# borodark/exmc

Hardware: AMD Instinct MI355X
Metric: leapfrog_steps_per_s (higher is better)
Workload: dtype f64; 1 GPU; eight_schools d=10, 4096 chains/GPU (4096 total), 138450 draws/chain (2769 steps of 50 draws) after one shared 1000-iteration warmup, max_tree_depth 10, target_accept 0.8; draws_per_chain=138450, lanes_per_chain=16, warmup_lanes_per_chain=16, seed=42

## Files before the change

exmc_amd/csrc/exmc_device.hpp:

```cpp
#pragma once

#include <hip/hip_runtime.h>
#include <stdint.h>
#include <type_traits>

#include <utility>

#include "../../include/exmc_detmath.h"

namespace exmc {

constexpr uint64_t kMask58 = (1ULL << 58) - 1;

__device__ __forceinline__ bool div_in_range(double x) {
  const uint32_t h = (uint32_t)__double2hiint(x) & 0x7fffffffu;
  return (h - 0x28300000u) < (0x57C00000u - 0x28300000u);
}

struct Recip {
  double b, r;
};

__device__ __forceinline__ Recip make_recip(double b) { return Recip{b, exmc_rcp_refined(b)}; }

__device__ __forceinline__ Recip make_recip_literal(double b) {
  __asm__ volatile("" : "+v"(b));
  return make_recip(b);
// ... 250 lines not shown
#define EXMC_SEQ2(I) EXMC_SEQ1(I) EXMC_FMAC_B(a1, v1, I)
#define EXMC_SEQ3(I) EXMC_SEQ2(I) EXMC_FMAC_B(a2, v2, I)
#define EXMC_SEQ6(I) EXMC_SEQ3(I) EXMC_FMAC_B(a3, v3, I) EXMC_FMAC_B(a4, v4, I) EXMC_FMAC_B(a5, v5, I)
#define EXMC_LANES_1(S) S(0)
#define EXMC_LANES_2(S) EXMC_LANES_1(S) S(1)
#define EXMC_LANES_3(S) EXMC_LANES_2(S) S(2)
#define EXMC_LANES_4(S) EXMC_LANES_3(S) S(3)
#define EXMC_LANES_5(S) EXMC_LANES_4(S) S(4)
#define EXMC_LANES_6(S) EXMC_LANES_5(S) S(5)
#define EXMC_LANES_7(S) EXMC_LANES_6(S) S(6)
#define EXMC_LANES_8(S) EXMC_LANES_7(S) S(7)
#define EXMC_LANES_9(S) EXMC_LANES_8(S) S(8)
#define EXMC_LANES_10(S) EXMC_LANES_9(S) S(9)
#define EXMC_LANES_11(S) EXMC_LANES_10(S) S(10)
#define EXMC_LANES_12(S) EXMC_LANES_11(S) S(11)
#define EXMC_SEQSUM_ASM(SEQ, OUTS, INS)                                                        \
  if constexpr (NL == 1) __asm__("s_nop 1\n\t" EXMC_LANES_1(SEQ) : OUTS : INS);                \
  else if constexpr (NL == 2) __asm__("s_nop 1\n\t" EXMC_LANES_2(SEQ) : OUTS : INS);           \
  else if constexpr (NL == 3) __asm__("s_nop 1\n\t" EXMC_LANES_3(SEQ) : OUTS : INS);           \
  else if constexpr (NL == 4) __asm__("s_nop 1\n\t" EXMC_LANES_4(SEQ) : OUTS : INS);           \
  else if constexpr (NL == 5) __asm__("s_nop 1\n\t" EXMC_LANES_5(SEQ) : OUTS : INS);           \
  else if constexpr (NL == 6) __asm__("s_nop 1\n\t" EXMC_LANES_6(SEQ) : OUTS : INS);           \
  else if constexpr (NL == 7) __asm__("s_nop 1\n\t" EXMC_LANES_7(SEQ) : OUTS : INS);           \
  else if constexpr (NL == 8) __asm__("s_nop 1\n\t" EXMC_LANES_8(SEQ) : OUTS : INS);           \
  else if constexpr (NL == 9) __asm__("s_nop 1\n\t" EXMC_LANES_9(SEQ) : OUTS : INS);           \
  else if constexpr (NL == 10) __asm__("s_nop 1\n\t" EXMC_LANES_10(SEQ) : OUTS : INS);         \
  else if constexpr (NL == 11) __asm__("s_nop 1\n\t" EXMC_LANES_11(SEQ) : OUTS : INS);         \
  else __asm__("s_nop 1\n\t" EXMC_LANES_12(SEQ) : OUTS : INS);
#define EXMC_COMMA ,

__device__ __forceinline__ double seq_one() { return 1.0; }

template <int NL>
__device__ __forceinline__ void row_seqsum(double& a0, double v0) {
  static_assert(NL >= 1 && NL <= 12, "lanes of one DPP row, where the chain beats the butterfly");
  const double one = seq_one();
  EXMC_SEQSUM_ASM(EXMC_SEQ1, [a0] "+v"(a0), [v0] "v"(v0) EXMC_COMMA [one] "v"(one))
}
template <int NL>
__device__ __forceinline__ void row_seqsum(double& a0, double& a1, double v0, double v1) {
  const double one = seq_one();
  EXMC_SEQSUM_ASM(EXMC_SEQ2, [a0] "+v"(a0) EXMC_COMMA [a1] "+v"(a1),
                  [v0] "v"(v0) EXMC_COMMA [v1] "v"(v1) EXMC_COMMA [one] "v"(one))
}
template <int NL>
__device__ __forceinline__ void row_seqsum(double& a0, double& a1, double& a2, double v0, double v1,
                                           double v2) {
  const double one = seq_one();
  EXMC_SEQSUM_ASM(EXMC_SEQ3, [a0] "+v"(a0) EXMC_COMMA [a1] "+v"(a1) EXMC_COMMA [a2] "+v"(a2),
                  [v0] "v"(v0) EXMC_COMMA [v1] "v"(v1) EXMC_COMMA [v2] "v"(v2) EXMC_COMMA [one] "v"(one))
}
#define EXMC_FMAC_R(A, V, I) \
  "v_fmac_f64_dpp %[" #A "], %[" #V "], %[one] row_newbcast:%[l" #I "] row_mask:0xf bank_mask:0xf\n\t"
#define EXMC_SEQ3R(I) EXMC_FMAC_R(a0, v0, I) EXMC_FMAC_R(a1, v1, I) EXMC_FMAC_R(a2, v2, I)
#define EXMC_LANE_R(I) [l##I] "n"((I0 + I) & 15)
template <int I0, int NL>
__device__ __forceinline__ void row_seqsum_lanes(double& a0, double& a1, double& a2, double v0, double v1,
                                                 double v2) {
  static_assert(I0 >= 0 && NL >= 1 && NL <= 12 && I0 + NL <= 16, "a lane range of one DPP row");
  const double one = seq_one();
  EXMC_SEQSUM_ASM(EXMC_SEQ3R, [a0] "+v"(a0) EXMC_COMMA [a1] "+v"(a1) EXMC_COMMA [a2] "+v"(a2),
                  [v0] "v"(v0) EXMC_COMMA [v1] "v"(v1) EXMC_COMMA [v2] "v"(v2) EXMC_COMMA [one] "v"(one) EXMC_COMMA
                  EXMC_LANE_R(0) EXMC_COMMA EXMC_LANE_R(1) EXMC_COMMA EXMC_LANE_R(2) EXMC_COMMA EXMC_LANE_R(3) EXMC_COMMA
                  EXMC_LANE_R(4) EXMC_COMMA EXMC_LANE_R(5) EXMC_COMMA EXMC_LANE_R(6) EXMC_COMMA EXMC_LANE_R(7) EXMC_COMMA
                  EXMC_LANE_R(8) EXMC_COMMA EXMC_LANE_R(9) EXMC_COMMA EXMC_LANE_R(10) EXMC_COMMA EXMC_LANE_R(11))
}
#ifndef EXMC_ROW_SUM_PIECES
#define EXMC_ROW_SUM_PIECES 7
#endif
#define EXMC_MV1(I) \
  "v_fmac_f64_dpp %[acc], %[x], %[c" #I "] row_newbcast:" #I " row_mask:0xf bank_mask:0xf\n\t"
template <int NL>
__device__ __forceinline__ double row_matvec(double x, const double (&c)[NL]) {
  static_assert(NL >= 1 && NL <= 12, "lanes of one DPP row");
  double acc = 0.0;
#define EXMC_MV_C(I) [c##I] "v"(c[(I) < NL ? (I) : 0])
  EXMC_SEQSUM_ASM(EXMC_MV1, [acc] "+v"(acc),
                  [x] "v"(x) EXMC_COMMA EXMC_MV_C(0) EXMC_COMMA EXMC_MV_C(1) EXMC_COMMA EXMC_MV_C(2) EXMC_COMMA
                  EXMC_MV_C(3) EXMC_COMMA EXMC_MV_C(4) EXMC_COMMA EXMC_MV_C(5) EXMC_COMMA EXMC_MV_C(6) EXMC_COMMA
                  EXMC_MV_C(7) EXMC_COMMA EXMC_MV_C(8) EXMC_COMMA EXMC_MV_C(9) EXMC_COMMA EXMC_MV_C(10) EXMC_COMMA
                  EXMC_MV_C(11))
#undef EXMC_MV_C
  return acc;
}
#define EXMC_OUTER1(I) \
  "v_fmac_f64_dpp %[m" #I "], %[x], %[c] row_newbcast:" #I " row_mask:0xf bank_mask:0xf\n\t"
template <int NL>
__device__ __forceinline__ void row_outer_acc(double (&m)[NL], double x, double c) {
  static_assert(NL >= 1 && NL <= 12, "lanes of one DPP row");
  double pad[12];
#pragma unroll
  for (int j = 0; j < 12; j++) pad[j] = (j < NL) ? m[j < NL ? j : 0] : 0.0;
#define EXMC_OUTER_M(I) [m##I] "+v"(pad[I])
  EXMC_SEQSUM_ASM(EXMC_OUTER1,
                  EXMC_OUTER_M(0) EXMC_COMMA EXMC_OUTER_M(1) EXMC_COMMA EXMC_OUTER_M(2) EXMC_COMMA EXMC_OUTER_M(3) EXMC_COMMA
                  EXMC_OUTER_M(4) EXMC_COMMA EXMC_OUTER_M(5) EXMC_COMMA EXMC_OUTER_M(6) EXMC_COMMA EXMC_OUTER_M(7) EXMC_COMMA
                  EXMC_OUTER_M(8) EXMC_COMMA EXMC_OUTER_M(9) EXMC_COMMA EXMC_OUTER_M(10) EXMC_COMMA EXMC_OUTER_M(11),
                  [x] "v"(x) EXMC_COMMA [c] "v"(c))
#undef EXMC_OUTER_M
#pragma unroll
  for (int j = 0; j < NL; j++) m[j] = pad[j];
}
template <int J>
__device__ __forceinline__ double row_bcast_f64(double x) {
  double acc = 0.0;
  const double one = seq_one();
  __asm__("s_nop 1\n\tv_fmac_f64_dpp %0, %1, %2 row_newbcast:%3 row_mask:0xf bank_mask:0xf"
          : "+v"(acc) : "v"(x), "v"(one), "n"(J));
  return acc;
}

template <int NL>
__device__ __forceinline__ void row_seqsum6(double (&a)[6], const double (&v)[6]) {
  const double one = seq_one();
  EXMC_SEQSUM_ASM(EXMC_SEQ6,
                  [a0] "+v"(a[0]) EXMC_COMMA [a1] "+v"(a[1]) EXMC_COMMA [a2] "+v"(a[2]) EXMC_COMMA
                  [a3] "+v"(a[3]) EXMC_COMMA [a4] "+v"(a[4]) EXMC_COMMA [a5] "+v"(a[5]),
                  [v0] "v"(v[0]) EXMC_COMMA [v1] "v"(v[1]) EXMC_COMMA [v2] "v"(v[2]) EXMC_COMMA
                  [v3] "v"(v[3]) EXMC_COMMA [v4] "v"(v[4]) EXMC_COMMA [v5] "v"(v[5]) EXMC_COMMA
                  [one] "v"(one))
}

template <int G>
__device__ __forceinline__ double group_bcast(double v, int src) {
  if (G == 1) return v;
  const int lane = threadIdx.x & 63;
  return __shfl(v, (lane & ~(G - 1)) | src, 64);
}

template <int G, int SRC>
__device__ __forceinline__ double group_bcast_c(double v) {
  static_assert(SRC >= 0 && SRC < G, "source lane outside the group");
  if constexpr (G == 1) {
    return v;
  } else if constexpr (G == 2) {
// ... 213 lines not shown
    const double mx = (a > b) ? a : b;
    if (mx == -exmc_from_bits(EXMC_INF_BITS) || mx == -1.0e300) return -1.0e300;
    const double mn = (a > b) ? b : a;
    return mx + log_ge1(1.0 + exp_le0(mn - mx));
  }
  __device__ static __forceinline__ double lse_arg(double a, double b) {
    return ((a > b) ? b : a) - ((a > b) ? a : b);
  }
  __device__ static __forceinline__ double lse_finish(double a, double b, double log1pe) {
    const double mx = (a > b) ? a : b;
    const bool none = (mx == -exmc_from_bits(EXMC_INF_BITS) || mx == -1.0e300);
    return none ? -1.0e300 : mx + log1pe;
  }
};

template <int CTRL>
__device__ __forceinline__ double xchg_dpp(double v) { return dpp_move<CTRL>(v); }
template <int PATTERN>
__device__ __forceinline__ double xchg_swizzle(double v) {
  return __hiloint2double(__builtin_amdgcn_ds_swizzle(__double2hiint(v), PATTERN),
                          __builtin_amdgcn_ds_swizzle(__double2loint(v), PATTERN));
}
__device__ __forceinline__ double xchg_xor4(double v) {
#if EXMC_XROW_PERMLANE
  return __hiloint2double(xor4_b32(__double2hiint(v)), xor4_b32(__double2loint(v)));
#else
  return xchg_swizzle<(4 << 10) | 0x1F>(v);
#endif
}
__device__ __forceinline__ double xchg_xor32(double v) {
// ... 133 lines not shown
#pragma unroll
  for (int k = 0; k < DPL; k++) {
    const double v = rho[k] * im[k];
    sa = valid[k] ? (sa + v * pa[k]) : sa;
    sb = valid[k] ? (sb + v * pb[k]) : sb;
  }
}

template <int G, int DPL, int D = G * DPL, bool kLds = false>
__device__ __forceinline__ bool uturn(const double (&rho)[DPL], const double (&pa)[DPL],
                                      const double (&pb)[DPL], const double (&im)[DPL],
                                      const bool (&valid)[DPL]) {
  double s[2];
  if constexpr (kSeqSum<G, D>) {
    const double v = rho[0] * im[0];
    s[0] = s[1] = 0.0;
    row_seqsum<D>(s[0], s[1], v * pa[0], v * pb[0]);
  } else {
    uturn_partials<DPL>(rho, pa, pb, im, valid, s[0], s[1]);
    if constexpr (G == 64 && (kLds || EXMC_XROW_PERMLANE)) {
      const unsigned long long neg = __ballot((rs64_reduce2(s) < 0.0) ? 1 : 0);
      return (neg & 0x3ULL) != 0;
    } else {
      group_allsum_n<G, 2, kLds>(s);
    }
  }
  return (s[0] < 0.0) || (s[1] < 0.0);
}

template <int G, int DPL, int D = G * DPL, bool kLds = false>
__device__ __forceinline__ void uturn3(const double (&r1)[DPL], const double (&a1)[DPL],
                                       const double (&b1)[DPL], const double (&r2)[DPL],
                                       const double (&a2)[DPL], const double (&b2)[DPL],
                                       const double (&r3)[DPL], const double (&a3)[DPL],
                                       const double (&b3)[DPL], const double (&im)[DPL],
                                       const bool (&valid)[DPL], bool& c1, bool& c23) {
  double s[6];
  if constexpr (kSeqSum<G, D>) {
    const double v1 = r1[0] * im[0], v2 = r2[0] * im[0], v3 = r3[0] * im[0];
    const double t[6] = {v1 * a1[0], v1 * b1[0], v2 * a2[0], v2 * b2[0], v3 * a3[0], v3 * b3[0]};
#pragma unroll
    for (int j = 0; j < 6; j++) s[j] = 0.0;
    row_seqsum6<D>(s, t);
  } else {
    uturn_partials<DPL>(r1, a1, b1, im, valid, s[0], s[1]);
    uturn_partials<DPL>(r2, a2, b2, im, valid, s[2], s[3]);
    uturn_partials<DPL>(r3, a3, b3, im, valid, s[4], s[5]);
    if constexpr (G == 64 && (kLds || EXMC_XROW_PERMLANE)) {
      const unsigned long long neg = __ballot((rs64_reduce6(s) < 0.0) ? 1 : 0);
      c1 = (neg & ((1ULL << 0) | (1ULL << 4))) != 0;
      c23 = (neg & ((1ULL << 1) | (1ULL << 2) | (1ULL << 3) | (1ULL << 5))) != 0;
      return;
    } else {
      group_allsum_n<G, 6, kLds>(s);
    }
  }
  c1 = (s[0] < 0.0) || (s[1] < 0.0);
  c23 = (s[2] < 0.0) || (s[3] < 0.0) || (s[4] < 0.0) || (s[5] < 0.0);
// ... 232 lines not shown
```

exmc_amd/csrc/exmc_hip.hip:

```cpp
#include "../../include/exmc_hip.h"
#include "../../include/exmc_hip_compare.h"
#include "../../include/exmc_hip_pathfinder.h"
#include "../../include/exmc_hip_advi.h"
#include "../../include/exmc_hip_predictive.h"
#include "../../include/exmc_hip_ppc.h"
#include "../../include/exmc_hip_loo_pit.h"
#include "../../include/exmc_hip_convergence.h"

#include <hip/hip_runtime.h>

#include <cmath>
#include <cstdio>
#include <cstdlib>
#include <cstring>
#include <algorithm>
#include <atomic>
#include <mutex>
#include <string>
#include <type_traits>
#include <unordered_map>
#include <vector>

#include "../../include/exmc_zig_tables.h"
#include "exmc_kernels.hpp"
// ... 20 lines not shown
  if (e != hipSuccess) return e;
  e = hipMemcpyToSymbol(HIP_SYMBOL(g_prof), z, sizeof(z));
  if (e != hipSuccess) return e;
  static const char* nm[9] = {"transition_start", "doubling_start", "leapfrog+model", "leaf",
                              "ascend", "outer_merge", "transition_done", "tree_prefix", "loop"};
  unsigned long long tot = 0;
  for (int i = 0; i < 9; i++) tot += h[i];
  fprintf(stderr, "[exmc prof] %s %.3f ms, passes (sum over waves) %llu, cycles %llu\n", what, ms, h[9], tot);
  for (int i = 0; i < 9; i++)
    if ((i != 7 || h[7]) && h[9])
      fprintf(stderr, "[exmc prof]   %-18s %6.1f%%  %8.1f cycles/pass\n", nm[i],
              100.0 * (double)h[i] / (double)tot, (double)h[i] / (double)h[9]);
  if (h[10])
    fprintf(stderr, "[exmc prof]   integrator wave: %llu units, %.1f cycles/unit compute, %.1f barrier wait, %.1f other\n",
            h[10], (double)h[11] / (double)h[10], (double)h[12] / (double)h[10], (double)h[13] / (double)h[10]);
  return hipSuccess;
}
#endif


const uint64_t kZigKi[256] = EXMC_ZIG_KI_INIT;
const double kZigWi[256] = EXMC_ZIG_WI_INIT;
const double kZigFi[256] = EXMC_ZIG_FI_INIT;


#ifdef EXMC_PLUGIN_MODULES
extern "C" const unsigned char* const exmc_blob_table[];
struct ModSet {
  int device = -1;
  std::vector<hipModule_t> mods;
// ... 2673 lines not shown
```

exmc_amd/csrc/exmc_models.hpp:

```cpp
#pragma once

#include "exmc_device.hpp"

namespace exmc {

__device__ __forceinline__ double clamp200(double z) { return fmax(-200.0, fmin(z, 200.0)); }

struct ModelDefaults {
  static constexpr bool kVregMath = false;
  static constexpr bool kCoop = false;
  static constexpr int kExtraLdsDoubles = 0;
  static constexpr int kStageDoubles = 0;
  template <class C>
  __host__ static bool stage_ok(const C&) { return true; }
  static constexpr int kStageRowOffset = 0;
  static constexpr int kLdsDataDoubles = 0;
  static constexpr bool kPipeWarmup = true;
  static constexpr bool kHasPipeWarmup = true;
  static constexpr bool kXRowLds = false;
  static constexpr bool kRowDense = false;
  static constexpr bool kLaneDense = false;
  static constexpr bool kDenseImage = false;
  static constexpr int kDenseLdsDoubles = 0;
  static constexpr int kNutsWavesPerSimd = 1;
// ... 3 lines not shown
  static constexpr int kPipeNutsLevels = 0;
  static constexpr bool kNutsZigInLds = true;
  static constexpr bool kRegradProposal = false;
  static constexpr int kWgWaves = 0;
  static constexpr int kWgLdsLevels = 1;
  static constexpr int kWgImageDoubles = 0;
  template <class C>
  __host__ __device__ static bool wg_ok(const C&) { return false; }
  static constexpr bool kLeafPairs = false;
  static constexpr bool kLeafPairExp = false;
  static constexpr bool kLeanMomentum = false;
  static constexpr bool kPassExpPairs = false;
  static constexpr bool kOuterLogPair = false;
  static constexpr bool kTreePrefix = false;
  static constexpr bool kRngWindow = false;
};

extern __shared__ double exmc_dyn_lds[];
typedef double exmc_v2d __attribute__((ext_vector_type(2)));
typedef __attribute__((address_space(3))) exmc_v2d lds_v2d;
typedef __attribute__((address_space(3))) double lds_f64_m;
static __device__ const double exmc_logtab_dev[2 * EXMC_LOGTAB_ENTRIES] = {EXMC_LOGTAB_VALUES};
__device__ static __forceinline__ double exmc_log_tab_global(double x) {
  double m;
  int e;
  const int i = exmc_logtab_split(x, &m, &e);
  return exmc_logtab_finish(m, e, exmc_logtab_dev[2 * i], exmc_logtab_dev[2 * i + 1]);
}

struct EightSchoolsConsts {
// ... 6 lines not shown
template <int G>
struct EightSchools : ModelDefaults {
  static constexpr int D = 10;
  static constexpr int DPL = (D + G - 1) / G;
  static constexpr bool kVregMath = (DPL <= 2);
#ifndef EXMC_ES_PIPE_LEVELS
#define EXMC_ES_PIPE_LEVELS 2
#endif
  static constexpr int kPipeNutsLevels = (G == 16) ? EXMC_ES_PIPE_LEVELS : 0;
  static constexpr bool kLeafPairs = (G == 16);
  static constexpr bool kLeafPairExp = (G == 16);
  static constexpr bool kLeanMomentum = (G == 16);
  static constexpr bool kOuterLogPair = (G == 16);
  static constexpr bool kTreePrefix = (G == 16);
  static constexpr bool kRngWindow = (G == 16);
  using MM = Math<kVregMath>;
  using Consts = EightSchoolsConsts;
  struct Lane {
    double y[DPL], lsg[DPL];
    Recip sg[DPL];
    Recip five;
    double cc;
  };

  __device__ static __forceinline__ void load(const Consts& c, int l, Lane& ln) {
#pragma unroll
    for (int k = 0; k < DPL; k++) {
      const int i = l + k * G;
      const int j = (i >= 2 && i < D) ? (i - 2) : 0;
      ln.y[k] = c.y[j];
// ... 30 lines not shown
    const double tau = MM::exp_pm200(zc);
    const bool isth = (l >= 2) && (l < D);
    const bool l0 = (l == 0), l1 = (l == 1);
    const double th = q[0];
    const double theta = mu + tau * th;
    const double resid = ln.y[0] - theta;
    constexpr bool kThetaLanes = (EXMC_ROW_SUM_PIECES & 1) != 0, kOneWatch = (EXMC_ROW_SUM_PIECES & 4) != 0;
    if constexpr (!kOneWatch) dv.watch_if(isth, resid);
    dv.watch_if(isth, ln.sg[0].b);
    const double z = dv(resid, ln.sg[0]);
    const double a = dv(z, ln.sg[0]);
    const double Lk = (-0.5 * (z * z)) - ln.lsg[0];
    const double Ak = a;
    const double Bk = a * th;
    double lik = 0.0, sa = 0.0, sb = 0.0;
    if constexpr (kThetaLanes) row_seqsum_lanes<2, D - 2>(lik, sa, sb, Lk, Ak, Bk);
    else row_seqsum<D>(lik, sa, sb, isth ? Lk : 0.0, isth ? Ak : 0.0, isth ? Bk : 0.0);
    const double x = l0 ? (mu - 0.0) : tau;
    if constexpr (kOneWatch) dv.watch_if(isth || l0, l0 ? x : resid);
    else dv.watch_if(l0, x);
    const double zh = dv(x, ln.five);
    const double zh2 = zh * zh;
    const double w = dv(zh, ln.five);
    const double den = 1.0 + zh2;
    const double dhc = -dv(2.0 * w, den);
    const bool in = (zraw > -200.0) && (zraw < 200.0);
    double g_tau = in ? ((dhc + sb) * tau + 1.0) : 0.0;
    __asm__("" : "+v"(g_tau));
    const double g_mu = (-w) + sa;
    const double g_th = (-th) + a * tau;
    const double u2 = l0 ? zh2 : (th * th);
// ... 1187 lines not shown
      if (j == J + 3) { T[k] = t_sy; g[k] = in_y ? ((dsy * sy + s[5]) + 1.0) : 0.0; }
      if (j == J + 4) { T[k] = -0.5 * (zb * zb + ln.kc[kN5]); g[k] = (-dv(zb, ln.five)) + s[4]; }
      if (j >= D) g[k] = 0.0;
    }
    return group_sum_slots<G, DPL>(T, valid, l, s[0]);
  }
};

template <class M>
struct RowDenseModel : M {
  static constexpr bool kRowDense = true;
  static constexpr bool kPipeWarmup = false;
  static constexpr bool kOuterLogPair = false;
  static constexpr bool kTreePrefix = false;
  static constexpr bool kRngWindow = false;
  static_assert(M::DPL == 1 && M::D <= 12, "row layout: one dimension per lane, D <= 12");
};

template <class M, int G>
struct LaneDenseModel : M {
  static constexpr bool kLaneDense = true;
  static constexpr bool kPipeWarmup = false;
  static constexpr int kNutsWavesPerSimd = 1;
  static constexpr int kPipeNutsLevels = 0;
  static constexpr bool kDenseImage = M::D * M::D * 8 <= 16 * 1024;
  static constexpr int kDenseLdsDoubles = (64 / G) * 3 * M::D + (kDenseImage ? M::D * M::D + 64 : 0);
  static_assert(G >= 16 && M::DPL * G >= M::D && !M::kCoop, "a lane layout that holds the whole chain");
};

}
// ... 446 lines not shown
```

exmc_amd/csrc/exmc_nuts.hpp:

```cpp
#pragma once

#include <type_traits>

#include "exmc_models.hpp"

#ifndef EXMC_ABLATE
#define EXMC_ABLATE 0
#endif

#ifndef EXMC_PROFILE_SECTIONS
#define EXMC_PROFILE_SECTIONS 0
#endif

namespace exmc {

#ifdef EXMC_XCC_PROBE
__device__ double g_wave_probe[4096 * 5];
#endif

#if EXMC_PROFILE_SECTIONS
__device__ unsigned long long g_prof[16];
#define EXMC_PROF_DECL long long prof_[10] = {0, 0, 0, 0, 0, 0, 0, 0, 0, 0}; long long prof_t_ = clock64();
#define EXMC_PROF(i) { const long long n_ = clock64(); prof_[i] += n_ - prof_t_; prof_t_ = n_; }
#define EXMC_PROF_COUNT(i) { prof_[i] += 1; }
#define EXMC_PROF_FLUSH                                                        \
  if ((threadIdx.x & 63) == 0) {                                               \
    for (int i_ = 0; i_ < 10; i_++) atomicAdd(&g_prof[i_], (unsigned long long)prof_[i_]); \
  }
#define EXMC_IPROF_DECL long long iprof_[4] = {0, 0, 0, 0}; long long iprof_t_ = clock64();
#define EXMC_IPROF(i) { const long long n_ = clock64(); iprof_[i] += n_ - iprof_t_; iprof_t_ = n_; }
#define EXMC_IPROF_COUNT { iprof_[0] += 1; }
#define EXMC_IPROF_FLUSH                                                       \
  if ((threadIdx.x & 63) == 0) {                                               \
    for (int i_ = 0; i_ < 4; i_++) atomicAdd(&g_prof[10 + i_], (unsigned long long)iprof_[i_]); \
  }
#else
#define EXMC_IPROF_DECL
#define EXMC_IPROF(i)
#define EXMC_IPROF_COUNT
#define EXMC_IPROF_FLUSH
#define EXMC_PROF_DECL
#define EXMC_PROF(i)
#define EXMC_PROF_COUNT(i)
#define EXMC_PROF_FLUSH
#endif

struct FlatOrder {
  const int32_t* perm = nullptr;
  const int32_t* rank = nullptr;
};

// ... 534 lines not shown
  __device__ __forceinline__ uint64_t next_rank() const {
    const uint32_t l = (uint32_t)__builtin_amdgcn_mov_dpp((int)lo, 0x100 + kOff + 1, 0xF, 0xF, true);
    const uint32_t h = (uint32_t)__builtin_amdgcn_mov_dpp((int)hi, 0x100 + kOff + 1, 0xF, 0xF, true);
    return ((uint64_t)h << 32) | (uint64_t)l;
  }
  __device__ __forceinline__ uint64_t at(int p) const {
    const int src = (((threadIdx.x & 63) & ~15) | (kOff + p)) << 2;
    const uint32_t l = (uint32_t)__builtin_amdgcn_ds_bpermute(src, (int)lo);
    const uint32_t h = (uint32_t)__builtin_amdgcn_ds_bpermute(src, (int)hi);
    return ((uint64_t)h << 32) | (uint64_t)l;
  }
};

template <class M, int G, int W>
__device__ __forceinline__ void draw_momentum_window(const NutsLane<M, G>& L, const RngRowWindow<W>& win,
                                                     Rng& rng, double (&z)[M::DPL], int& left) {
  constexpr int D = M::D;
  static_assert(G == 16 && M::DPL == 1, "a group is one DPP row with one dimension a lane");
  static_assert(W >= D + 2, "the state behind the momentum at shift 0");
  constexpr int kMaxShift = W - D - 2;
  const int base = (threadIdx.x & 63) & ~(G - 1);
  const int rank = L.rank[0];
  z[0] = 0.0;
  int pos = 0, shift = 0;
  left = D;
  uint64_t la = 0, lb = 0;
  bool flat = true;
  for (;;) {
    const bool live = L.valid[0] && (rank >= pos);
    const uint64_t w = flat ? win.next_rank() : win.at(live ? 1 + rank + shift : 0);
    double zz;
    const bool acc = normal_fast(rng_scramble(w), L.zt, zz);
    const bool fail = live && !acc;
    z[0] = (live && acc) ? zz : z[0];
    const unsigned long long m = __ballot(fail ? 1 : 0);
    const unsigned long long gm = (m >> base) & ((1ULL << G) - 1ULL);
    const int j = (gm != 0) ? (__ffsll((long long)gm) - 1) : D;
    if (m == 0) break;
    flat = false;
    if (j < D) {
      const int pj = 1 + j + shift;
      Rng rj;
      rj.a = win.at(pj - 1);
      rj.b = win.at(pj);
      int words = 0;
      zz = rng_normal_counted(rj, L.zt, L.nor_r, words);
      z[0] = (rank == j) ? zz : z[0];
      shift += words - 1;
      pos = j + 1;
      if (shift > kMaxShift) {
        la = rj.a;
        lb = rj.b;
        left = pos;
        pos = D;
      }
    } else {
      pos = D;
    }
  }
  if (flat) {
    rng = win.template state<D + 1>();
  } else {
    const bool gone = shift > kMaxShift;
    const int pe = gone ? 1 : D + 1 + shift;
    const uint64_t ea = win.at(pe - 1), eb = win.at(pe);
    rng.a = gone ? la : ea;
    rng.b = gone ? lb : eb;
  }
}

template <class M, int G>
__device__ __forceinline__ void draw_momentum_variates(const NutsLane<M, G>& L, Rng& rng,
                                                       double (&z)[M::DPL]) {
// ... 767 lines not shown
    t_rho[k] = t_qp[k] = t_gp[k] = c_rho[k] = c_pin[k] = c_qp[k] = c_gp[k] = 0.0;
  }
  double t_logpP = 0.0, t_lsw = 0.0, t_acc = 0.0, jlp0 = 0.0;
  int t_n = 0, t_depth = 0;
  bool t_div = false, t_turn = false, go_right = true;
  double eps_dir = eps;
  Rng trng = st.rng;
  const bool has = L.alive;
  constexpr bool kPrefix = M::kTreePrefix && M::kLeafPairs && Pipe::kTreePrefix && EXMC_ABLATE == 0;
  constexpr bool kWindow = kPrefix && M::kRngWindow && G == 16 && EXMC_RNG_WINDOW_STAGE >= 1;
  constexpr bool kWinMomentum = kWindow && EXMC_RNG_WINDOW_STAGE >= 2 && DPL == 1 && M::kLeanMomentum && !M::kRowDense;
  using Win = RngRowWindow<kWinMomentum ? EXMC_RNG_WINDOW : 11>;
  Win win{0, 0};

  EXMC_PROF_DECL
  for (int draw = 0; draw < n_draws; draw++) {
    EXMC_PROF(8)
    bool alive = has;
    bool have_z = false;
    double z_pre[DPL];
#pragma unroll
    for (int k = 0; k < DPL; k++) z_pre[k] = 0.0;
    if constexpr (Pipe::kOn) {
      if (pipe->pending) {
        pipe->sync();
        pipe->pending = false;
        have_z = pipe->take_momentum(st.rng, z_pre);
      }
    }
    if (has) {
      if (have_z) {
        momentum_from_variates<M, G>(L, z_pre, pL);
      } else if (kWinMomentum && L.perm == nullptr) {
        if constexpr (kWinMomentum) {
          int left = 0;
          if (draw > 0) draw_momentum_window<M, G>(L, win, st.rng, z_pre, left);
          if (draw == 0 || __any((left < M::D) ? 1 : 0) != 0)
            draw_momentum_lean_from<M, G>(L, st.rng, z_pre, left, draw == 0);
          momentum_from_variates<M, G>(L, z_pre, pL);
        }
      } else {
        draw_momentum<M, G>(L, st.rng, pL);
      }
      jlp0 = st.logp - mass_ke<M, G>(L, pL);
      trng = st.rng;
#pragma unroll
      for (int k = 0; k < DPL; k++) {
        qL[k] = qR[k] = t_qp[k] = st.q[k];
        gL[k] = gR[k] = t_gp[k] = st.g[k];
        pR[k] = t_rho[k] = pL[k];
      }
      t_logpP = st.logp;
      t_lsw = 0.0;
      t_acc = 0.0;
      t_n = 0;
      t_div = t_turn = false;
      t_depth = 0;
    }
    if constexpr (Pipe::kOn) {
// ... 321 lines not shown
    if constexpr (Pipe::kOn) pipe->pending = true;
    if constexpr (kRegrad) {
      (void)M::logp_grad(mc, L.ln, l, t_qp, t_gp);
    }
    if (has) {
      if constexpr (kWindow) st.rng = win.template state<1>();
      else (void)rng_uniform(st.rng);
      st.logp = t_logpP;
#pragma unroll
      for (int k = 0; k < DPL; k++) { st.q[k] = t_qp[k]; st.g[k] = t_gp[k]; }
      sink(draw, st.q, st.logp, t_depth, t_n, t_div, t_acc, jlp0);
    }
    EXMC_PROF(6)
  }
  EXMC_PROF_FLUSH
}

template <class M, int G>
__device__ __forceinline__ void rowdense_load(NutsLane<M, G>& L, const double* cov, const double* chol,
                                              int stride) {
  constexpr int D = M::D;
  const int i = L.l < D ? L.l : 0;
#pragma unroll
  for (int j = 0; j < (M::kRowDense ? D : 1); j++) {
    L.rd.cr[j] = cov ? cov[(size_t)(i * D + j) * stride] : ((i == j) ? 1.0 : 0.0);
    L.rd.ncc[j] = (chol && j > i) ? -chol[(size_t)(j * D + i) * stride] : 0.0;
  }
  L.rd.diag = chol ? chol[(size_t)(i * D + i) * stride] : 1.0;
}

// ... 135 lines not shown
  unsigned long long lf_total = 0, div_total = 0;
  int n_published = 0;
  const int l = L.l;
  struct Cursor {
    char* p;
    long long step;
  };
  auto cursor = [&](void* base, bool mine, size_t elem, size_t index, size_t row_elems) -> Cursor {
    const bool on = (base != nullptr) && mine;
    return Cursor{on ? (char*)base + index * elem : (char*)P.scratch,
                  on ? (long long)(row_elems * elem) : 0LL};
  };
  const bool own = (l == 0);
  Cursor c_draw[DPL];
  Cursor c_logp, c_depth, c_steps, c_div, c_acc, c_energy;
  auto bind = [&](int ch, size_t row) {
    const size_t stat0 = row * C + ch;
#pragma unroll
    for (int k = 0; k < DPL; k++)
      c_draw[k] = cursor(P.tr.draws, L.valid[k], 8, (row * D + (l + k * G)) * C + ch, (size_t)D * C);
    c_logp = cursor(P.tr.logp, own, 8, stat0, C);
    c_depth = cursor(P.tr.tree_depth, own, 4, stat0, C);
    c_steps = cursor(P.tr.n_steps, own, 4, stat0, C);
    c_div = cursor(P.tr.divergent, own, 4, stat0, C);
    c_acc = cursor(P.tr.accept_prob, own, 8, stat0, C);
    c_energy = cursor(P.tr.energy, own, 8, stat0, C);
  };
  bind(chain, (size_t)P.draw_offset);
  auto sink = [&](int, const double (&sq)[DPL], double slogp, int depth, int t_n, bool t_div,
                  double t_acc, double jlp0) {
#pragma unroll
    for (int k = 0; k < DPL; k++) {
      if (L.valid[k]) *(double*)c_draw[k].p = sq[k];
      c_draw[k].p += c_draw[k].step;
    }
    if (own) {
      *(double*)c_logp.p = slogp;
      *(int32_t*)c_depth.p = depth;
      *(int32_t*)c_steps.p = t_n;
      *(int32_t*)c_div.p = t_div ? 1 : 0;
      *(double*)c_acc.p = (t_n > 0) ? (t_acc / (double)t_n) : 0.0;
      *(double*)c_energy.p = -jlp0;
    }
    c_logp.p += c_logp.step;
    c_depth.p += c_depth.step;
    c_steps.p += c_steps.step;
    c_div.p += c_div.step;
    c_acc.p += c_acc.step;
    c_energy.p += c_energy.step;
    lf_total += (unsigned long long)t_n;
    div_total += t_div ? 1u : 0u;
    if constexpr (kStream) {
      __builtin_amdgcn_fence(__ATOMIC_RELEASE, "");
      n_published++;
      if (tid == 0) __hip_atomic_store(P.progress, n_published, __ATOMIC_RELAXED, __HIP_MEMORY_SCOPE_SYSTEM);
    }
  };
#ifdef EXMC_XCC_PROBE
  const long long wave_c0 = clock64(), wave_w0 = wall_clock64();
  auto probe_out = [&]() {
    if constexpr (kPipe) {
      if (lane == 0 && 2 * blockIdx.x + (threadIdx.x >> 6) < 4096) {
        double* const e = g_wave_probe + (2 * blockIdx.x + (threadIdx.x >> 6)) * 5;
        e[2] = (double)lf_total;
// ... 136 lines not shown
        atomicAdd(&P.counters[0], lf_total);
        atomicAdd(&P.counters[1], div_total);
      }
#ifdef EXMC_XCC_PROBE
      probe_out();
#endif
      return;
    }
    nuts_run<M, G, LDSL>(mc, L, st, P.n_draws, P.eps, P.max_depth, sink);
  } else {
    nuts_run<M, G, LDSL>(mc, L, st, P.n_draws, P.eps, P.max_depth, sink);
  }
#ifdef EXMC_XCC_PROBE
  probe_out();
#endif

  if (!has_chain) return;
  chain_store<M, G>(P.st, C, chain, l, st);
  if (l == 0 && P.counters) {
    atomicAdd(&P.counters[0], lf_total);
    atomicAdd(&P.counters[1], div_total);
  }
}

template <class M, int LDSL, int W>
__host__ __device__ constexpr size_t nuts_wg_extra_offset() {
  return (size_t)W * LDSL * nuts_nslot<M>() * kNutsBlock + kZigLdsBytes / 8;
}
template <class M, int LDSL, int W>
__host__ __device__ constexpr size_t nuts_wg_image_offset() {
// ... 760 lines not shown
```

Baseline: 3.803 billion leapfrog_steps/s.

## Spread per-draw trace stores across spare lanes, fold zeroing into DPP sums, single-pass wedge normal

The draw sink now has the six spare lanes of each 16-lane row (lanes D..D+5) write the per-draw statistics, one value per lane, instead of lane 0 issuing six serial stores. The seq-sum DPP blocks zero their accumulators inside the asm block with v_mov_b64, replacing separate zeroing moves plus a nop. Momentum redraws in the RNG window try one ziggurat wedge attempt before falling back to the full counted normal. Profiling subsection counters are also added behind compile flags. All three speed paths are on by default through EXMC_FIXED_PART_PIECES=7, so a wrong lane-to-stream mapping or a change in the RNG word count could break correctness.

```diff
diff --git a/exmc_amd/csrc/exmc_device.hpp b/exmc_amd/csrc/exmc_device.hpp
--- a/exmc_amd/csrc/exmc_device.hpp
+++ b/exmc_amd/csrc/exmc_device.hpp
@@ -11,6 +11,10 @@
 namespace exmc {
 
 constexpr uint64_t kMask58 = (1ULL << 58) - 1;
+
+#ifndef EXMC_FIXED_PART_PIECES
+#define EXMC_FIXED_PART_PIECES 7
+#endif
 
 __device__ __forceinline__ bool div_in_range(double x) {
   const uint32_t h = (uint32_t)__double2hiint(x) & 0x7fffffffu;
@@ -291,19 +295,20 @@
 #define EXMC_LANES_10(S) EXMC_LANES_9(S) S(9)
 #define EXMC_LANES_11(S) EXMC_LANES_10(S) S(10)
 #define EXMC_LANES_12(S) EXMC_LANES_11(S) S(11)
-#define EXMC_SEQSUM_ASM(SEQ, OUTS, INS)                                                        \
-  if constexpr (NL == 1) __asm__("s_nop 1\n\t" EXMC_LANES_1(SEQ) : OUTS : INS);                \
-  else if constexpr (NL == 2) __asm__("s_nop 1\n\t" EXMC_LANES_2(SEQ) : OUTS : INS);           \
-  else if constexpr (NL == 3) __asm__("s_nop 1\n\t" EXMC_LANES_3(SEQ) : OUTS : INS);           \
-  else if constexpr (NL == 4) __asm__("s_nop 1\n\t" EXMC_LANES_4(SEQ) : OUTS : INS);           \
-  else if constexpr (NL == 5) __asm__("s_nop 1\n\t" EXMC_LANES_5(SEQ) : OUTS : INS);           \
-  else if constexpr (NL == 6) __asm__("s_nop 1\n\t" EXMC_LANES_6(SEQ) : OUTS : INS);           \
-  else if constexpr (NL == 7) __asm__("s_nop 1\n\t" EXMC_LANES_7(SEQ) : OUTS : INS);           \
-  else if constexpr (NL == 8) __asm__("s_nop 1\n\t" EXMC_LANES_8(SEQ) : OUTS : INS);           \
-  else if constexpr (NL == 9) __asm__("s_nop 1\n\t" EXMC_LANES_9(SEQ) : OUTS : INS);           \
-  else if constexpr (NL == 10) __asm__("s_nop 1\n\t" EXMC_LANES_10(SEQ) : OUTS : INS);         \
-  else if constexpr (NL == 11) __asm__("s_nop 1\n\t" EXMC_LANES_11(SEQ) : OUTS : INS);         \
-  else __asm__("s_nop 1\n\t" EXMC_LANES_12(SEQ) : OUTS : INS);
+#define EXMC_SEQSUM_ASM_H(HEAD, SEQ, OUTS, INS)                                              \
+  if constexpr (NL == 1) __asm__(HEAD EXMC_LANES_1(SEQ) : OUTS : INS);                         \
+  else if constexpr (NL == 2) __asm__(HEAD EXMC_LANES_2(SEQ) : OUTS : INS);                    \
+  else if constexpr (NL == 3) __asm__(HEAD EXMC_LANES_3(SEQ) : OUTS : INS);                    \
+  else if constexpr (NL == 4) __asm__(HEAD EXMC_LANES_4(SEQ) : OUTS : INS);                    \
+  else if constexpr (NL == 5) __asm__(HEAD EXMC_LANES_5(SEQ) : OUTS : INS);                    \
+  else if constexpr (NL == 6) __asm__(HEAD EXMC_LANES_6(SEQ) : OUTS : INS);                    \
+  else if constexpr (NL == 7) __asm__(HEAD EXMC_LANES_7(SEQ) : OUTS : INS);                    \
+  else if constexpr (NL == 8) __asm__(HEAD EXMC_LANES_8(SEQ) : OUTS : INS);                    \
+  else if constexpr (NL == 9) __asm__(HEAD EXMC_LANES_9(SEQ) : OUTS : INS);                    \
+  else if constexpr (NL == 10) __asm__(HEAD EXMC_LANES_10(SEQ) : OUTS : INS);                  \
+  else if constexpr (NL == 11) __asm__(HEAD EXMC_LANES_11(SEQ) : OUTS : INS);                  \
+  else __asm__(HEAD EXMC_LANES_12(SEQ) : OUTS : INS);
+#define EXMC_NOP2 "s_nop 1\n\t"
 #define EXMC_COMMA ,
 
 __device__ __forceinline__ double seq_one() { return 1.0; }
@@ -312,19 +317,19 @@
 __device__ __forceinline__ void row_seqsum(double& a0, double v0) {
   static_assert(NL >= 1 && NL <= 12, "lanes of one DPP row, where the chain beats the butterfly");
   const double one = seq_one();
-  EXMC_SEQSUM_ASM(EXMC_SEQ1, [a0] "+v"(a0), [v0] "v"(v0) EXMC_COMMA [one] "v"(one))
+  EXMC_SEQSUM_ASM_H(EXMC_NOP2, EXMC_SEQ1, [a0] "+v"(a0), [v0] "v"(v0) EXMC_COMMA [one] "v"(one))
 }
 template <int NL>
 __device__ __forceinline__ void row_seqsum(double& a0, double& a1, double v0, double v1) {
   const double one = seq_one();
-  EXMC_SEQSUM_ASM(EXMC_SEQ2, [a0] "+v"(a0) EXMC_COMMA [a1] "+v"(a1),
+  EXMC_SEQSUM_ASM_H(EXMC_NOP2, EXMC_SEQ2, [a0] "+v"(a0) EXMC_COMMA [a1] "+v"(a1),
                   [v0] "v"(v0) EXMC_COMMA [v1] "v"(v1) EXMC_COMMA [one] "v"(one))
 }
 template <int NL>
 __device__ __forceinline__ void row_seqsum(double& a0, double& a1, double& a2, double v0, double v1,
                                            double v2) {
   const double one = seq_one();
-  EXMC_SEQSUM_ASM(EXMC_SEQ3, [a0] "+v"(a0) EXMC_COMMA [a1] "+v"(a1) EXMC_COMMA [a2] "+v"(a2),
+  EXMC_SEQSUM_ASM_H(EXMC_NOP2, EXMC_SEQ3, [a0] "+v"(a0) EXMC_COMMA [a1] "+v"(a1) EXMC_COMMA [a2] "+v"(a2),
                   [v0] "v"(v0) EXMC_COMMA [v1] "v"(v1) EXMC_COMMA [v2] "v"(v2) EXMC_COMMA [one] "v"(one))
 }
 #define EXMC_FMAC_R(A, V, I) \
@@ -336,7 +341,7 @@
                                                  double v2) {
   static_assert(I0 >= 0 && NL >= 1 && NL <= 12 && I0 + NL <= 16, "a lane range of one DPP row");
   const double one = seq_one();
-  EXMC_SEQSUM_ASM(EXMC_SEQ3R, [a0] "+v"(a0) EXMC_COMMA [a1] "+v"(a1) EXMC_COMMA [a2] "+v"(a2),
+  EXMC_SEQSUM_ASM_H(EXMC_NOP2, EXMC_SEQ3R, [a0] "+v"(a0) EXMC_COMMA [a1] "+v"(a1) EXMC_COMMA [a2] "+v"(a2),
                   [v0] "v"(v0) EXMC_COMMA [v1] "v"(v1) EXMC_COMMA [v2] "v"(v2) EXMC_COMMA [one] "v"(one) EXMC_COMMA
                   EXMC_LANE_R(0) EXMC_COMMA EXMC_LANE_R(1) EXMC_COMMA EXMC_LANE_R(2) EXMC_COMMA EXMC_LANE_R(3) EXMC_COMMA
                   EXMC_LANE_R(4) EXMC_COMMA EXMC_LANE_R(5) EXMC_COMMA EXMC_LANE_R(6) EXMC_COMMA EXMC_LANE_R(7) EXMC_COMMA
@@ -345,6 +350,35 @@
 #ifndef EXMC_ROW_SUM_PIECES
 #define EXMC_ROW_SUM_PIECES 7
 #endif
+#define EXMC_ZERO_B(A) "v_mov_b64 %[" #A "], 0\n\t"
+inline constexpr bool kZeroInBlock = (EXMC_FIXED_PART_PIECES & 4) != 0;
+template <int NL>
+__device__ __forceinline__ void row_seqsum_zero(double& a0, double& a1, double v0, double v1) {
+  if constexpr (kZeroInBlock) {
+    const double one = seq_one();
+    EXMC_SEQSUM_ASM_H(EXMC_ZERO_B(a0) EXMC_ZERO_B(a1), EXMC_SEQ2, [a0] "=&v"(a0) EXMC_COMMA [a1] "=&v"(a1),
+                      [v0] "v"(v0) EXMC_COMMA [v1] "v"(v1) EXMC_COMMA [one] "v"(one))
+  } else {
+    a0 = a1 = 0.0;
+    row_seqsum<NL>(a0, a1, v0, v1);
+  }
+}
+template <int I0, int NL>
+__device__ __forceinline__ void row_seqsum_lanes_zero(double& a0, double& a1, double& a2, double v0, double v1,
+                                                      double v2) {
+  if constexpr (kZeroInBlock) {
+    const double one = seq_one();
+    EXMC_SEQSUM_ASM_H(EXMC_ZERO_B(a0) EXMC_ZERO_B(a1) EXMC_ZERO_B(a2), EXMC_SEQ3R,
+                      [a0] "=&v"(a0) EXMC_COMMA [a1] "=&v"(a1) EXMC_COMMA [a2] "=&v"(a2),
+                      [v0] "v"(v0) EXMC_COMMA [v1] "v"(v1) EXMC_COMMA [v2] "v"(v2) EXMC_COMMA [one] "v"(one) EXMC_COMMA
+                      EXMC_LANE_R(0) EXMC_COMMA EXMC_LANE_R(1) EXMC_COMMA EXMC_LANE_R(2) EXMC_COMMA EXMC_LANE_R(3) EXMC_COMMA
+                      EXMC_LANE_R(4) EXMC_COMMA EXMC_LANE_R(5) EXMC_COMMA EXMC_LANE_R(6) EXMC_COMMA EXMC_LANE_R(7) EXMC_COMMA
+                      EXMC_LANE_R(8) EXMC_COMMA EXMC_LANE_R(9) EXMC_COMMA EXMC_LANE_R(10) EXMC_COMMA EXMC_LANE_R(11))
+  } else {
+    a0 = a1 = a2 = 0.0;
+    row_seqsum_lanes<I0, NL>(a0, a1, a2, v0, v1, v2);
+  }
+}
 #define EXMC_MV1(I) \
   "v_fmac_f64_dpp %[acc], %[x], %[c" #I "] row_newbcast:" #I " row_mask:0xf bank_mask:0xf\n\t"
 template <int NL>
@@ -352,7 +386,7 @@
   static_assert(NL >= 1 && NL <= 12, "lanes of one DPP row");
   double acc = 0.0;
 #define EXMC_MV_C(I) [c##I] "v"(c[(I) < NL ? (I) : 0])
-  EXMC_SEQSUM_ASM(EXMC_MV1, [acc] "+v"(acc),
+  EXMC_SEQSUM_ASM_H(EXMC_NOP2, EXMC_MV1, [acc] "+v"(acc),
                   [x] "v"(x) EXMC_COMMA EXMC_MV_C(0) EXMC_COMMA EXMC_MV_C(1) EXMC_COMMA EXMC_MV_C(2) EXMC_COMMA
                   EXMC_MV_C(3) EXMC_COMMA EXMC_MV_C(4) EXMC_COMMA EXMC_MV_C(5) EXMC_COMMA EXMC_MV_C(6) EXMC_COMMA
                   EXMC_MV_C(7) EXMC_COMMA EXMC_MV_C(8) EXMC_COMMA EXMC_MV_C(9) EXMC_COMMA EXMC_MV_C(10) EXMC_COMMA
@@ -369,7 +403,7 @@
 #pragma unroll
   for (int j = 0; j < 12; j++) pad[j] = (j < NL) ? m[j < NL ? j : 0] : 0.0;
 #define EXMC_OUTER_M(I) [m##I] "+v"(pad[I])
-  EXMC_SEQSUM_ASM(EXMC_OUTER1,
+  EXMC_SEQSUM_ASM_H(EXMC_NOP2, EXMC_OUTER1,
                   EXMC_OUTER_M(0) EXMC_COMMA EXMC_OUTER_M(1) EXMC_COMMA EXMC_OUTER_M(2) EXMC_COMMA EXMC_OUTER_M(3) EXMC_COMMA
                   EXMC_OUTER_M(4) EXMC_COMMA EXMC_OUTER_M(5) EXMC_COMMA EXMC_OUTER_M(6) EXMC_COMMA EXMC_OUTER_M(7) EXMC_COMMA
                   EXMC_OUTER_M(8) EXMC_COMMA EXMC_OUTER_M(9) EXMC_COMMA EXMC_OUTER_M(10) EXMC_COMMA EXMC_OUTER_M(11),
@@ -390,12 +424,29 @@
 template <int NL>
 __device__ __forceinline__ void row_seqsum6(double (&a)[6], const double (&v)[6]) {
   const double one = seq_one();
-  EXMC_SEQSUM_ASM(EXMC_SEQ6,
+  EXMC_SEQSUM_ASM_H(EXMC_NOP2, EXMC_SEQ6,
                   [a0] "+v"(a[0]) EXMC_COMMA [a1] "+v"(a[1]) EXMC_COMMA [a2] "+v"(a[2]) EXMC_COMMA
                   [a3] "+v"(a[3]) EXMC_COMMA [a4] "+v"(a[4]) EXMC_COMMA [a5] "+v"(a[5]),
                   [v0] "v"(v[0]) EXMC_COMMA [v1] "v"(v[1]) EXMC_COMMA [v2] "v"(v[2]) EXMC_COMMA
                   [v3] "v"(v[3]) EXMC_COMMA [v4] "v"(v[4]) EXMC_COMMA [v5] "v"(v[5]) EXMC_COMMA
                   [one] "v"(one))
+}
+template <int NL>
+__device__ __forceinline__ void row_seqsum6_zero(double (&a)[6], const double (&v)[6]) {
+  if constexpr (kZeroInBlock) {
+    const double one = seq_one();
+    EXMC_SEQSUM_ASM_H(EXMC_ZERO_B(a0) EXMC_ZERO_B(a1) EXMC_ZERO_B(a2) EXMC_ZERO_B(a3) EXMC_ZERO_B(a4) EXMC_ZERO_B(a5),
+                      EXMC_SEQ6,
+                      [a0] "=&v"(a[0]) EXMC_COMMA [a1] "=&v"(a[1]) EXMC_COMMA [a2] "=&v"(a[2]) EXMC_COMMA
+                      [a3] "=&v"(a[3]) EXMC_COMMA [a4] "=&v"(a[4]) EXMC_COMMA [a5] "=&v"(a[5]),
+                      [v0] "v"(v[0]) EXMC_COMMA [v1] "v"(v[1]) EXMC_COMMA [v2] "v"(v[2]) EXMC_COMMA
+                      [v3] "v"(v[3]) EXMC_COMMA [v4] "v"(v[4]) EXMC_COMMA [v5] "v"(v[5]) EXMC_COMMA
+                      [one] "v"(one))
+  } else {
+#pragma unroll
+    for (int j = 0; j < 6; j++) a[j] = 0.0;
+    row_seqsum6<NL>(a, v);
+  }
 }
 
 template <int G>
@@ -639,6 +690,35 @@
   }
 };
 
+template <bool kVreg>
+__device__ __forceinline__ double normal_wedge_once(uint64_t w, Rng& r, const ZigTables& zt, double nor_r,
+                                                    int& words) {
+  const int sign = (int)((w >> 6) & 1);
+  const uint64_t R = w >> 7;
+  const int idx = (int)(R & 255);
+  double x = (double)R * zt.wi[idx];
+  if (sign) x = -x;
+  Rng r2 = r;
+  rng_advance(r2);
+  const double u0 = rng_uniform(r2);
+  const int ix = (idx != 0) ? idx : 1;
+  const double fi2 = zt.fi[ix];
+  const bool acc = (idx != 0) && ((zt.fi[ix - 1] - fi2) * u0 + fi2 < Math<kVreg>::exp_le0(-0.5 * x * x));
+  double z = x;
+  int n = 2;
+  if (__any(acc ? 0 : 1) != 0) {
+    if (!acc) {
+      Rng rr = (idx != 0) ? r2 : r;
+      n = (idx != 0) ? 2 : 0;
+      z = rng_normal_counted(rr, zt, nor_r, n);
+      r2 = rr;
+    }
+  }
+  r = r2;
+  words += n;
+  return z;
+}
+
 template <int CTRL>
 __device__ __forceinline__ double xchg_dpp(double v) { return dpp_move<CTRL>(v); }
 template <int PATTERN>
@@ -802,8 +882,7 @@
   double s[2];
   if constexpr (kSeqSum<G, D>) {
     const double v = rho[0] * im[0];
-    s[0] = s[1] = 0.0;
-    row_seqsum<D>(s[0], s[1], v * pa[0], v * pb[0]);
+    row_seqsum_zero<D>(s[0], s[1], v * pa[0], v * pb[0]);
   } else {
     uturn_partials<DPL>(rho, pa, pb, im, valid, s[0], s[1]);
     if constexpr (G == 64 && (kLds || EXMC_XROW_PERMLANE)) {
@@ -827,9 +906,7 @@
   if constexpr (kSeqSum<G, D>) {
     const double v1 = r1[0] * im[0], v2 = r2[0] * im[0], v3 = r3[0] * im[0];
     const double t[6] = {v1 * a1[0], v1 * b1[0], v2 * a2[0], v2 * b2[0], v3 * a3[0], v3 * b3[0]};
-#pragma unroll
-    for (int j = 0; j < 6; j++) s[j] = 0.0;
-    row_seqsum6<D>(s, t);
+    row_seqsum6_zero<D>(s, t);
   } else {
     uturn_partials<DPL>(r1, a1, b1, im, valid, s[0], s[1]);
     uturn_partials<DPL>(r2, a2, b2, im, valid, s[2], s[3]);
diff --git a/exmc_amd/csrc/exmc_hip.hip b/exmc_amd/csrc/exmc_hip.hip
--- a/exmc_amd/csrc/exmc_hip.hip
+++ b/exmc_amd/csrc/exmc_hip.hip
@@ -58,6 +58,27 @@
   if (h[10])
     fprintf(stderr, "[exmc prof]   integrator wave: %llu units, %.1f cycles/unit compute, %.1f barrier wait, %.1f other\n",
             h[10], (double)h[11] / (double)h[10], (double)h[12] / (double)h[10], (double)h[13] / (double)h[10]);
+#if EXMC_PROFILE_SECTIONS >= 2
+  unsigned long long s[8], sz[8] = {0};
+  e = hipMemcpyFromSymbol(s, HIP_SYMBOL(g_prof_sub), sizeof(s));
+  if (e != hipSuccess) return e;
+  e = hipMemcpyToSymbol(HIP_SYMBOL(g_prof_sub), sz, sizeof(sz));
+  if (e != hipSuccess) return e;
+#if EXMC_PROFILE_SECTIONS == 2
+  static const char* sn[5] = {"start: window draw", "start: long-way rounds", "start: stepping loop",
+                              "start: momentum_from_variates", "start: mass_ke"};
+  const int ns = 5;
+#else
+  static const char* sn[3] = {"done: draws store", "done: stat stores", "done: cursor steps"};
+  const int ns = 3;
+#endif
+  for (int i = 0; i < ns; i++)
+    if (h[9])
+      fprintf(stderr, "[exmc prof]   %-30s %6.2f%%  %8.1f cycles/pass\n", sn[i],
+              100.0 * (double)s[i] / (double)tot, (double)s[i] / (double)h[9]);
+  if (EXMC_PROFILE_SECTIONS == 2)
+    fprintf(stderr, "[exmc prof]   long-way rounds (sum over waves) %llu, wave-transitions %llu\n", s[5], s[6]);
+#endif
   return hipSuccess;
 }
 #endif
diff --git a/exmc_amd/csrc/exmc_models.hpp b/exmc_amd/csrc/exmc_models.hpp
--- a/exmc_amd/csrc/exmc_models.hpp
+++ b/exmc_amd/csrc/exmc_models.hpp
@@ -41,6 +41,7 @@
   static constexpr bool kOuterLogPair = false;
   static constexpr bool kTreePrefix = false;
   static constexpr bool kRngWindow = false;
+  static constexpr bool kPackedTrace = false;
 };
 
 extern __shared__ double exmc_dyn_lds[];
@@ -77,6 +78,7 @@
   static constexpr bool kOuterLogPair = (G == 16);
   static constexpr bool kTreePrefix = (G == 16);
   static constexpr bool kRngWindow = (G == 16);
+  static constexpr bool kPackedTrace = (G == 16);
   using MM = Math<kVregMath>;
   using Consts = EightSchoolsConsts;
   struct Lane {
@@ -137,7 +139,7 @@
     const double Ak = a;
     const double Bk = a * th;
     double lik = 0.0, sa = 0.0, sb = 0.0;
-    if constexpr (kThetaLanes) row_seqsum_lanes<2, D - 2>(lik, sa, sb, Lk, Ak, Bk);
+    if constexpr (kThetaLanes) row_seqsum_lanes_zero<2, D - 2>(lik, sa, sb, Lk, Ak, Bk);
     else row_seqsum<D>(lik, sa, sb, isth ? Lk : 0.0, isth ? Ak : 0.0, isth ? Bk : 0.0);
     const double x = l0 ? (mu - 0.0) : tau;
     if constexpr (kOneWatch) dv.watch_if(isth || l0, l0 ? x : resid);
@@ -1355,6 +1357,7 @@
   static constexpr bool kOuterLogPair = false;
   static constexpr bool kTreePrefix = false;
   static constexpr bool kRngWindow = false;
+  static constexpr bool kPackedTrace = false;
   static_assert(M::DPL == 1 && M::D <= 12, "row layout: one dimension per lane, D <= 12");
 };
 
diff --git a/exmc_amd/csrc/exmc_nuts.hpp b/exmc_amd/csrc/exmc_nuts.hpp
--- a/exmc_amd/csrc/exmc_nuts.hpp
+++ b/exmc_amd/csrc/exmc_nuts.hpp
@@ -34,7 +34,30 @@
   if ((threadIdx.x & 63) == 0) {                                               \
     for (int i_ = 0; i_ < 4; i_++) atomicAdd(&g_prof[10 + i_], (unsigned long long)iprof_[i_]); \
   }
+__device__ unsigned long long g_prof_sub[8];
+#define EXMC_SUBPROF_DECL long long sub_[8] = {0, 0, 0, 0, 0, 0, 0, 0};
+#define EXMC_SUBPROF_FLUSH                                                     \
+  if ((threadIdx.x & 63) == 0) {                                               \
+    for (int i_ = 0; i_ < 8; i_++) atomicAdd(&g_prof_sub[i_], (unsigned long long)sub_[i_]); \
+  }
+#if EXMC_PROFILE_SECTIONS == 2
+#define EXMC_SUBPROF(i) { const long long n_ = clock64(); sub_[i] += n_ - prof_t_; prof_t_ = n_; }
 #else
+#define EXMC_SUBPROF(i)
+#endif
+#if EXMC_PROFILE_SECTIONS == 3
+#define EXMC_SINKPROF_T0 long long sink_t_ = clock64();
+#define EXMC_SINKPROF(i) { const long long n_ = clock64(); sub_[i] += n_ - sink_t_; sink_t_ = n_; }
+#else
+#define EXMC_SINKPROF_T0
+#define EXMC_SINKPROF(i)
+#endif
+#else
+#define EXMC_SUBPROF_DECL
+#define EXMC_SUBPROF_FLUSH
+#define EXMC_SUBPROF(i)
+#define EXMC_SINKPROF_T0
+#define EXMC_SINKPROF(i)
 #define EXMC_IPROF_DECL
 #define EXMC_IPROF(i)
 #define EXMC_IPROF_COUNT
@@ -599,7 +622,8 @@
 
 template <class M, int G, int W>
 __device__ __forceinline__ void draw_momentum_window(const NutsLane<M, G>& L, const RngRowWindow<W>& win,
-                                                     Rng& rng, double (&z)[M::DPL], int& left) {
+                                                     Rng& rng, double (&z)[M::DPL], int& left,
+                                                     long long* prof_long = nullptr) {
   constexpr int D = M::D;
   static_assert(G == 16 && M::DPL == 1, "a group is one DPP row with one dimension a lane");
   static_assert(W >= D + 2, "the state behind the momentum at shift 0");
@@ -623,13 +647,19 @@
     const int j = (gm != 0) ? (__ffsll((long long)gm) - 1) : D;
     if (m == 0) break;
     flat = false;
+#if EXMC_PROFILE_SECTIONS == 2
+    const long long long_t0 = clock64();
+#endif
     if (j < D) {
       const int pj = 1 + j + shift;
       Rng rj;
       rj.a = win.at(pj - 1);
       rj.b = win.at(pj);
       int words = 0;
-      zz = rng_normal_counted(rj, L.zt, L.nor_r, words);
+      if constexpr ((EXMC_FIXED_PART_PIECES & 2) != 0)
+        zz = normal_wedge_once<M::kVregMath>(rng_scramble(rj.b), rj, L.zt, L.nor_r, words);
+      else
+        zz = rng_normal_counted(rj, L.zt, L.nor_r, words);
       z[0] = (rank == j) ? zz : z[0];
       shift += words - 1;
       pos = j + 1;
@@ -642,6 +672,12 @@
     } else {
       pos = D;
     }
+#if EXMC_PROFILE_SECTIONS == 2
+    if (prof_long) {
+      prof_long[0] += clock64() - long_t0;
+      prof_long[1] += 1;
+    }
+#endif
   }
   if (flat) {
     rng = win.template state<D + 1>();
@@ -1439,8 +1475,12 @@
   Win win{0, 0};
 
   EXMC_PROF_DECL
+  EXMC_SUBPROF_DECL
   for (int draw = 0; draw < n_draws; draw++) {
     EXMC_PROF(8)
+#if EXMC_PROFILE_SECTIONS == 2
+    sub_[6] += 1;
+#endif
     bool alive = has;
     bool have_z = false;
     double z_pre[DPL];
@@ -1459,15 +1499,29 @@
       } else if (kWinMomentum && L.perm == nullptr) {
         if constexpr (kWinMomentum) {
           int left = 0;
+#if EXMC_PROFILE_SECTIONS == 2
+          if (draw > 0) {
+            long long lw[2] = {0, 0};
+            draw_momentum_window<M, G>(L, win, st.rng, z_pre, left, lw);
+            EXMC_SUBPROF(0)
+            sub_[0] -= lw[0];
+            sub_[1] += lw[0];
+            sub_[5] += lw[1];
+          }
+#else
           if (draw > 0) draw_momentum_window<M, G>(L, win, st.rng, z_pre, left);
+#endif
           if (draw == 0 || __any((left < M::D) ? 1 : 0) != 0)
             draw_momentum_lean_from<M, G>(L, st.rng, z_pre, left, draw == 0);
+          EXMC_SUBPROF(2)
           momentum_from_variates<M, G>(L, z_pre, pL);
+          EXMC_SUBPROF(3)
         }
       } else {
         draw_momentum<M, G>(L, st.rng, pL);
       }
       jlp0 = st.logp - mass_ke<M, G>(L, pL);
+      EXMC_SUBPROF(4)
       trng = st.rng;
 #pragma unroll
       for (int k = 0; k < DPL; k++) {
@@ -1819,6 +1873,9 @@
     EXMC_PROF(6)
   }
   EXMC_PROF_FLUSH
+#if EXMC_PROFILE_SECTIONS == 2
+  EXMC_SUBPROF_FLUSH
+#endif
 }
 
 template <class M, int G>
@@ -1984,40 +2041,80 @@
   const bool own = (l == 0);
   Cursor c_draw[DPL];
   Cursor c_logp, c_depth, c_steps, c_div, c_acc, c_energy;
+  constexpr bool kPacked = M::kPackedTrace && (EXMC_FIXED_PART_PIECES & 1) != 0;
+  static_assert(!M::kPackedTrace || (DPL == 1 && G - D >= 6), "six spare lanes behind one dimension a lane");
+  Cursor c8{nullptr, 0}, c4{nullptr, 0};
+  int on_bits = 0;
   auto bind = [&](int ch, size_t row) {
     const size_t stat0 = row * C + ch;
-#pragma unroll
-    for (int k = 0; k < DPL; k++)
-      c_draw[k] = cursor(P.tr.draws, L.valid[k], 8, (row * D + (l + k * G)) * C + ch, (size_t)D * C);
-    c_logp = cursor(P.tr.logp, own, 8, stat0, C);
-    c_depth = cursor(P.tr.tree_depth, own, 4, stat0, C);
-    c_steps = cursor(P.tr.n_steps, own, 4, stat0, C);
-    c_div = cursor(P.tr.divergent, own, 4, stat0, C);
-    c_acc = cursor(P.tr.accept_prob, own, 8, stat0, C);
-    c_energy = cursor(P.tr.energy, own, 8, stat0, C);
+    if constexpr (kPacked) {
+      void* const b8 = (l < D) ? (void*)P.tr.draws
+                     : (l == D) ? (void*)P.tr.accept_prob
+                     : (l == D + 1) ? (void*)P.tr.logp
+                     : (l == D + 2) ? (void*)P.tr.energy : nullptr;
+      void* const b4 = (l == D + 3) ? (void*)P.tr.tree_depth
+                     : (l == D + 4) ? (void*)P.tr.n_steps
+                     : (l == D + 5) ? (void*)P.tr.divergent : nullptr;
+      on_bits = (b8 != nullptr ? 1 : 0) | (b4 != nullptr ? 2 : 0);
+      c8 = cursor(b8, true, 8, (l < D) ? (row * D + l) * C + ch : stat0, (l < D) ? (size_t)D * C : (size_t)C);
+      c4 = cursor(b4, true, 4, stat0, C);
+    } else {
+#pragma unroll
+      for (int k = 0; k < DPL; k++)
+        c_draw[k] = cursor(P.tr.draws, L.valid[k], 8, (row * D + (l + k * G)) * C + ch, (size_t)D * C);
+      c_logp = cursor(P.tr.logp, own, 8, stat0, C);
+      c_depth = cursor(P.tr.tree_depth, own, 4, stat0, C);
+      c_steps = cursor(P.tr.n_steps, own, 4, stat0, C);
+      c_div = cursor(P.tr.divergent, own, 4, stat0, C);
+      c_acc = cursor(P.tr.accept_prob, own, 8, stat0, C);
+      c_energy = cursor(P.tr.energy, own, 8, stat0, C);
+    }
   };
   bind(chain, (size_t)P.draw_offset);
+  EXMC_SUBPROF_DECL
   auto sink = [&](int, const double (&sq)[DPL], double slogp, int depth, int t_n, bool t_div,
                   double t_acc, double jlp0) {
-#pragma unroll
-    for (int k = 0; k < DPL; k++) {
-      if (L.valid[k]) *(double*)c_draw[k].p = sq[k];
-      c_draw[k].p += c_draw[k].step;
-    }
-    if (own) {
-      *(double*)c_logp.p = slogp;
-      *(int32_t*)c_depth.p = depth;
-      *(int32_t*)c_steps.p = t_n;
-      *(int32_t*)c_div.p = t_div ? 1 : 0;
-      *(double*)c_acc.p = (t_n > 0) ? (t_acc / (double)t_n) : 0.0;
-      *(double*)c_energy.p = -jlp0;
-    }
-    c_logp.p += c_logp.step;
-    c_depth.p += c_depth.step;
-    c_steps.p += c_steps.step;
-    c_div.p += c_div.step;
-    c_acc.p += c_acc.step;
-    c_energy.p += c_energy.step;
+    EXMC_SINKPROF_T0
+    if constexpr (kPacked) {
+      double acc = (t_n > 0) ? (t_acc / (double)t_n) : 0.0, energy = -jlp0;
+      int32_t dv = t_div ? 1 : 0;
+      int lr = l, on = on_bits;
+      __asm__ volatile("" : "+v"(acc), "+v"(energy), "+v"(dv), "+v"(lr), "+v"(on));
+      const double s8 = (lr == D) ? acc : ((lr == D + 1) ? slogp : energy);
+      const double v8 = (lr < D) ? sq[0] : s8;
+      const int32_t s4 = (lr == D + 3) ? depth : dv;
+      const int32_t v4 = (lr == D + 4) ? t_n : s4;
+      if ((on & 1) != 0) *(double*)c8.p = v8;
+      EXMC_SINKPROF(0)
+      if ((on & 2) != 0) *(int32_t*)c4.p = v4;
+      EXMC_SINKPROF(1)
+      c8.p += c8.step;
+      c4.p += c4.step;
+      EXMC_SINKPROF(2)
+    } else {
+#pragma unroll
+      for (int k = 0; k < DPL; k++) {
+        if (L.valid[k]) *(double*)c_draw[k].p = sq[k];
+        c_draw[k].p += c_draw[k].step;
+      }
+      EXMC_SINKPROF(0)
+      if (own) {
+        *(double*)c_logp.p = slogp;
+        *(int32_t*)c_depth.p = depth;
+        *(int32_t*)c_steps.p = t_n;
+        *(int32_t*)c_div.p = t_div ? 1 : 0;
+        *(double*)c_acc.p = (t_n > 0) ? (t_acc / (double)t_n) : 0.0;
+        *(double*)c_energy.p = -jlp0;
+      }
+      EXMC_SINKPROF(1)
+      c_logp.p += c_logp.step;
+      c_depth.p += c_depth.step;
+      c_steps.p += c_steps.step;
+      c_div.p += c_div.step;
+      c_acc.p += c_acc.step;
+      c_energy.p += c_energy.step;
+      EXMC_SINKPROF(2)
+    }
     lf_total += (unsigned long long)t_n;
     div_total += t_div ? 1u : 0u;
     if constexpr (kStream) {
@@ -2184,6 +2281,9 @@
 #ifdef EXMC_XCC_PROBE
   probe_out();
 #endif
+#if EXMC_PROFILE_SECTIONS == 3
+  EXMC_SUBPROF_FLUSH
+#endif
 
   if (!has_chain) return;
   chain_store<M, G>(P.st, C, chain, l, st);
```

Result: faster. 3.864 billion leapfrog_steps/s, median of 6 (+1.6%).
